# pyannote/pyannote-audio

Hardware: AMD Instinct MI355X
Metric: audio-hours/sec (real-time factor) for speaker-diarization-3.1 pipeline (higher is better)
Workload: dtype f32

## Files before the change

include/pyannote_amd.h:

```cpp
#ifndef PYANNOTE_AMD_H
#define PYANNOTE_AMD_H

#include <stddef.h>
#include <stdint.h>

#ifdef __cplusplus
extern "C" {
#endif

int pa_version(void);
const char* pa_last_error(void);

void pa_prof_enable(int on);
size_t pa_prof_report(char* buf, size_t cap);

#define PA_MAX_LSTM_LAYERS 8
#define PA_MAX_LINEAR 4

typedef struct pa_seg_weights {
  int32_t sinc_stride;
  int32_t lstm_layers;
  int32_t lstm_hidden;
  int32_t lstm_bidir;
  int32_t num_linear;
// ... 27 lines not shown
                   int num_chunks, int num_samples, float* logp, uint8_t* multilabel, void* workspace,
                   size_t workspace_bytes, void* stream);

size_t pa_seg_files_workspace_bytes(const pa_seg_weights* w, int num_files, const int* chunks_per_file,
                                    int num_samples, int64_t chunk_stride);
int pa_seg_forward_files(const pa_seg_weights* w, const float* const* wavs, const int64_t* wav_lens,
                         const int* chunks_per_file, int num_files, int64_t chunk_stride, int num_samples,
                         float* logp, uint8_t* multilabel, void* workspace, size_t workspace_bytes, void* stream);

int pa_row_stats(const float* x, long row_stride, long total_len, int rows, int len, float eps,
                 float* mean, float* rstd, void* stream);
int pa_sinc_fir_pool(const float* wav, long wav_len, long chunk_stride, int B, int N, int stride,
                     const float* mean, const float* rstd, float gamma, float beta,
                     const float* filt_packed, float* out, void* stream);
int pa_sinc_fir_span(const float* wav, long wav_len, long span, const float* filt_packed, float* S, void* stream);
int pa_sinc_fix_pool(const float* S, long Pc, int positions_per_chunk_step, int B, int P, const float* mean,
                     const float* rstd, float gamma, float beta, const float* filt_packed, float* tap_sums,
                     float* out, void* stream);
int pa_sinc_fir_span_centred(const float* wav, long wav_len, long span, const float* mean0, const float* rstd0,
                             const float* filt_packed, float* S, void* stream);
int pa_sinc_fix_pool_centred(const float* S, long Pc, int positions_per_chunk_step, int B, int P, const float* wav,
                             long wav_len, int N, const float* mean, const float* rstd, float gamma, float beta,
                             const float* filt_packed, float* tap_sums, float* out, void* stream);
int pa_conv5_pool(const float* xin, int B, int cin, int Lin, const float* in_mean,
                  const float* in_rstd, const float* gam, const float* bet, const float* w_packed,
                  const float* bias64, float* out, void* stream);
int pa_norm_transpose(const float* xin, int B, int T, const float* in_mean, const float* in_rstd,
                      const float* gam, const float* bet, float* X0, void* stream);
int pa_gemm_tn_ex(const float* A, int lda, const float* W, int ldw, const float* bias, const float* Res,
                  float* C, long ldc, int M, int N, int K, int act, int out_mode, void* stream);
int pa_gemm_tn(const float* A, int lda, const float* W, int ldw, const float* bias, float* C, long ldc,
               int M, int N, int K, int act, int out_mode, void* stream);
int pa_gemm_tn_s2(const float* X, int B, int H, int W, int cin, const float* Wt, int ldw, const float* bias, float* C,
                  long ldc, int N, void* stream);
int pa_lstm_rec(const float* xproj, const float* whh_packed, float* out, int ntiles, int ndir, int T,
                void* stream);
int pa_lstm_rec_h(const float* xproj, const float* whh_packed, float* out, int ntiles, int ndir, int T, int H,
                  void* stream);
int pa_classifier(const float* X, int ldx, int K, int ntiles, int T, int B, const float* cw,
                  const float* cb, int NC, const unsigned char* mapping, int S, float* logp,
                  unsigned char* multilabel, void* stream);

#define PA_MAX_RES_BLOCKS 128

typedef struct pa_emb_weights {
  int32_t num_mel;
// ... 384 lines not shown
```

pyannote-audio_amd/csrc/forward_common.cpp:

```cpp
#include "forward_common.h"

#include <stdlib.h>

namespace pa {

bool sincnet_frames(int sinc_stride, int N, SincNetPlan* p) {
  p->L1 = (N - 251) / sinc_stride + 1;
  if (N < 251 || p->L1 < 3) return false;
  p->P1 = p->L1 / 3;
  if (p->P1 < 5) return false;
  p->P2 = (p->P1 - 4) / 3;
  if (p->P2 < 5) return false;
  p->T = (p->P2 - 4) / 3;
  return p->T >= 1;
}

bool sincnet_plan(int sinc_stride, int B, int N, Bump* ws, SincNetPlan* p) {
  if (!sincnet_frames(sinc_stride, N, p)) return false;
  p->wav_mean = ws->take(B);
  p->wav_rstd = ws->take(B);
  p->s1 = ws->take((size_t)B * 80 * p->P1);
  p->st1m = ws->take((size_t)B * 80);
  p->st1r = ws->take((size_t)B * 80);
  p->s2 = ws->take((size_t)B * 60 * p->P2);
// ... 4 lines not shown
  p->st3r = ws->take((size_t)B * 60);
  p->span = p->span_pos = 0;
  p->span_s = p->tap_sums = 0;
  return true;
}

void sincnet_plan_span(int sinc_stride, int B, int N, int64_t chunk_stride, Bump* ws, SincNetPlan* p) {
  const char* e = getenv("PA_SEG_SHARED_SINC");
  if ((e == nullptr || atoi(e) != 0) && sinc_stride == 10 && B >= 2 && chunk_stride > 0 && chunk_stride < N &&
      chunk_stride % 10 == 0 && (int64_t)(B - 1) * chunk_stride + N <= 0x7fffffffLL) {
    p->span = (long)(B - 1) * chunk_stride + N;
    p->span_pos = (p->span - 251) / 10 + 1;
    p->span_s = ws->take((size_t)80 * p->span_pos);
    p->tap_sums = ws->take(80);
  }
}

int sincnet_sinc_stage(const SincNetView& w, const SincNetPlan& p, const float* wav, int64_t wav_len,
                       int64_t chunk_stride, int B, int N, float* ws, void* stream) {
  PA_RUN(pa_row_stats(wav, chunk_stride, wav_len, B, N, 1e-5f, ws + p.wav_mean, ws + p.wav_rstd, stream));
  if (p.span_pos > 0) {
    PA_RUN(pa_sinc_fir_span_centred(wav, wav_len, p.span, ws + p.wav_mean, ws + p.wav_rstd, w.sinc_filt,
                                    ws + p.span_s, stream));
    PA_RUN(pa_sinc_fix_pool_centred(ws + p.span_s, p.span_pos, (int)(chunk_stride / 10), B, p.P1, wav, wav_len, N,
                                    ws + p.wav_mean, ws + p.wav_rstd, w.wav_gamma, w.wav_beta, w.sinc_filt,
                                    ws + p.tap_sums, ws + p.s1, stream));
  } else {
    PA_RUN(pa_sinc_fir_pool(wav, wav_len, chunk_stride, B, N, w.sinc_stride, ws + p.wav_mean, ws + p.wav_rstd,
                            w.wav_gamma, w.wav_beta, w.sinc_filt, ws + p.s1, stream));
  }
  return 0;
}

int sincnet_after_sinc(const SincNetView& w, const SincNetPlan& p, int B, float* ws, float* x0, void* stream) {
  PA_RUN(pa_row_stats(ws + p.s1, p.P1, (long)B * 80 * p.P1, B * 80, p.P1, 1e-5f, ws + p.st1m, ws + p.st1r, stream));
  PA_RUN(pa_conv5_pool(ws + p.s1, B, 80, p.P1, ws + p.st1m, ws + p.st1r, w.norm0, w.norm0 + 80, w.conv1_w, w.conv1_b,
                       ws + p.s2, stream));
  PA_RUN(pa_row_stats(ws + p.s2, p.P2, (long)B * 60 * p.P2, B * 60, p.P2, 1e-5f, ws + p.st2m, ws + p.st2r, stream));
  PA_RUN(pa_conv5_pool(ws + p.s2, B, 60, p.P2, ws + p.st2m, ws + p.st2r, w.norm1, w.norm1 + 60, w.conv2_w, w.conv2_b,
                       ws + p.s3, stream));
  PA_RUN(pa_row_stats(ws + p.s3, p.T, (long)B * 60 * p.T, B * 60, p.T, 1e-5f, ws + p.st3m, ws + p.st3r, stream));
  return pa_norm_transpose(ws + p.s3, B, p.T, ws + p.st3m, ws + p.st3r, w.norm2, w.norm2 + 60, x0, stream);
}

int sincnet_run(const SincNetView& w, const SincNetPlan& p, const float* wav, int64_t wav_len, int64_t chunk_stride,
                int B, int N, float* ws, float* x0, void* stream) {
  PA_RUN(sincnet_sinc_stage(w, p, wav, wav_len, chunk_stride, B, N, ws, stream));
  return sincnet_after_sinc(w, p, B, ws, x0, stream);
}

bool lstm_head_check(const LstmHeadView& w, const char* who) {
  if (w.lstm_hidden < 16 || w.lstm_hidden % 16 != 0 || w.lstm_hidden > 512 ||
      (!w.lstm_bidir && w.lstm_hidden % 32 != 0) || w.lstm_layers < 1 || w.lstm_layers > PA_MAX_LSTM_LAYERS ||
      w.num_linear > PA_MAX_LINEAR || (w.num_linear > 0 && (w.linear_hidden < 32 || w.linear_hidden % 32 != 0))) {
    set_error("%s: LSTM hidden size must be a multiple of 16 (32 when unidirectional) up to 512, "
              "Linear widths multiples of 32 (got %d, %d)", who, w.lstm_hidden, w.linear_hidden);
    return false;
  }
  return true;
}

void lstm_head_plan(const LstmHeadView& w, int B, int T, Bump* ws, LstmHeadPlan* p) {
  p->ntiles = num_tiles(B);
  p->M = tile_rows(B, T);
  const size_t nd = w.lstm_bidir ? 2 : 1, Hh = (size_t)w.lstm_hidden;
  const size_t lw = w.num_linear > 0 ? (size_t)w.linear_hidden : 0;
  p->xproj = ws->take((size_t)p->M * nd * 4 * Hh);
  p->h0 = ws->take((size_t)p->M * nd * Hh);
  p->h1 = ws->take((size_t)p->M * nd * Hh);
  p->l0 = ws->take((size_t)p->M * lw);
  p->l1 = ws->take((size_t)p->M * lw);
// ... 27 lines not shown
```

pyannote-audio_amd/csrc/forward_common.h:

```cpp
#pragma once
#include <hip/hip_runtime.h>
#include <stdint.h>

#include "../../include/pyannote_amd.h"
#include "common.h"

#define PA_RUN(call)                \
  do {                              \
    const int rc__ = (call);        \
    if (rc__ != 0) return rc__;     \
  } while (0)

namespace pa {

struct Bump {
  size_t o = 0;
  static size_t align(size_t n) { return (n + 63) & ~(size_t)63; }
  size_t take(size_t n) {
    const size_t r = o;
    o += align(n);
    return r;
  }
};

// ... 2 lines not shown

struct SincNetView {
  int sinc_stride;
  float wav_gamma, wav_beta;
  const float *sinc_filt, *norm0, *conv1_w, *conv1_b, *norm1, *conv2_w, *conv2_b, *norm2;
};
template <class W>
SincNetView sincnet_of(const W* w) {
  return {w->sinc_stride, w->wav_gamma, w->wav_beta, w->sinc_filt, w->norm0, w->conv1_w,
          w->conv1_b,     w->norm1,     w->conv2_w,  w->conv2_b,   w->norm2};
}

struct SincNetPlan {
  int L1, P1, P2, T;
  size_t wav_mean, wav_rstd, s1, st1m, st1r, s2, st2m, st2r, s3, st3m, st3r;
  long span, span_pos;
  size_t span_s, tap_sums;
};
PA_INTERNAL bool sincnet_frames(int sinc_stride, int N, SincNetPlan* p);
PA_INTERNAL bool sincnet_plan(int sinc_stride, int B, int N, Bump* ws, SincNetPlan* p);
PA_INTERNAL void sincnet_plan_span(int sinc_stride, int B, int N, int64_t chunk_stride, Bump* ws, SincNetPlan* p);
PA_INTERNAL int sincnet_sinc_stage(const SincNetView& w, const SincNetPlan& p, const float* wav, int64_t wav_len,
                                   int64_t chunk_stride, int B, int N, float* ws, void* stream);
PA_INTERNAL int sincnet_after_sinc(const SincNetView& w, const SincNetPlan& p, int B, float* ws, float* x0,
                                   void* stream);
PA_INTERNAL int sincnet_run(const SincNetView& w, const SincNetPlan& p, const float* wav, int64_t wav_len,
                            int64_t chunk_stride, int B, int N, float* ws, float* x0, void* stream);

struct LstmHeadView {
  int lstm_layers, lstm_hidden, lstm_bidir, num_linear, linear_hidden, num_classes, num_speakers;
  const float* const* lstm_wih;
  const float* const* lstm_bias;
  const float* const* lstm_whh;
  const float* const* lin_w;
  const float* const* lin_b;
  const float *cls_w, *cls_b;
  const uint8_t* powerset_map;
};
template <class W>
LstmHeadView lstm_head_of(const W* w) {
  return {w->lstm_layers, w->lstm_hidden, w->lstm_bidir, w->num_linear, w->linear_hidden, w->num_classes,
          w->num_speakers, w->lstm_wih,   w->lstm_bias,  w->lstm_whh,   w->lin_w,         w->lin_b,
          w->cls_w,        w->cls_b,      w->powerset_map};
}

struct LstmHeadPlan {
  int ntiles;
  long M;
// ... 9 lines not shown
```

pyannote-audio_amd/csrc/seg_forward.cpp:

```cpp
#include "forward_common.h"

namespace {

struct SegPlan {
  pa::SincNetPlan sinc;
  pa::LstmHeadPlan head;
  size_t x0, total;
};

bool make_plan(const pa_seg_weights* w, int B, int N, int64_t chunk_stride, SegPlan* p) {
  pa::Bump ws;
  if (!pa::sincnet_plan(w->sinc_stride, B, N, &ws, &p->sinc)) return false;
  p->x0 = ws.take((size_t)pa::tile_rows(B, p->sinc.T) * 64);
  pa::lstm_head_plan(pa::lstm_head_of(w), B, p->sinc.T, &ws, &p->head);
  pa::sincnet_plan_span(w->sinc_stride, B, N, chunk_stride, &ws, &p->sinc);
  p->total = ws.o;
  return true;
}

struct FilesPlan {
  SegPlan seg;
  long chunks;
  size_t span_base;
};
// ... 86 lines not shown
                         float* logp, uint8_t* multilabel, void* workspace, size_t workspace_bytes, void* stream) {
  FilesPlan p;
  const int bad = make_files_plan(w, num_files, chunks_per_file, num_samples, chunk_stride, &p);
  if (bad == 1) {
    pa::set_error("pa_seg_forward_files: a negative chunk count, or more than 65535 chunks in one launch group");
    return 3;
  }
  if (bad != 0) {
    pa::set_error("pa_seg_forward_files: chunk of %d samples is too short for SincNet", num_samples);
    return 3;
  }
  if (p.chunks == 0) return 0;
  const pa::LstmHeadView head = pa::lstm_head_of(w);
  if (!pa::lstm_head_check(head, "pa_seg_forward_files")) return 3;
  if (workspace_bytes < p.seg.total * sizeof(float)) {
    pa::set_error("pa_seg_forward_files: workspace too small (%zu < %zu bytes)", workspace_bytes,
                  p.seg.total * sizeof(float));
    return 3;
  }
  float* ws = (float*)workspace;
  const pa::SincNetView sinc = pa::sincnet_of(w);
  const int B = (int)p.chunks;
  long c0 = 0;
  for (int f = 0; f < num_files; ++f) {
    const int Bf = chunks_per_file[f];
    if (Bf == 0) continue;
    pa::SincNetPlan one = p.seg.sinc;
    one.wav_mean += c0;
    one.wav_rstd += c0;
    one.s1 += (size_t)c0 * 80 * one.P1;
    plan_file_span(w, Bf, num_samples, chunk_stride, p.span_base, &one);
    PA_RUN(pa::sincnet_sinc_stage(sinc, one, wavs[f], wav_lens[f], chunk_stride, Bf, num_samples, ws, stream));
    c0 += Bf;
  }
  PA_RUN(pa::sincnet_after_sinc(sinc, p.seg.sinc, B, ws, ws + p.seg.x0, stream));
  return pa::lstm_head_run(head, p.seg.head, ws + p.seg.x0, 64, B, p.seg.sinc.T, ws, logp, multilabel, stream);
}

}
```

pyannote-audio_amd/csrc/seg_frontend.hip:

```cpp
#include "common.h"

namespace pa {

__global__ __launch_bounds__(256) void k_row_stats(const float* __restrict__ x, long row_stride,
                                                    long total_len, int len, float eps,
                                                    float* __restrict__ mean_out,
                                                    float* __restrict__ rstd_out) {
  __shared__ float red[4];
  const long base = (long)blockIdx.x * row_stride;
  long avail = total_len - base;
  int valid = avail >= len ? len : (avail > 0 ? (int)avail : 0);
  const float* row = x + base;
  float s = 0.f;
  for (int i = threadIdx.x; i < valid; i += 256) s += row[i];
  const float mean = block_sum<4>(s, red) / (float)len;
  float q = 0.f;
  for (int i = threadIdx.x; i < valid; i += 256) {
    float d = row[i] - mean;
    q += d * d;
  }
  float var = block_sum<4>(q, red);
  var += (float)(len - valid) * mean * mean;
  var /= (float)len;
  if (threadIdx.x == 0) {
    mean_out[blockIdx.x] = mean;
    rstd_out[blockIdx.x] = 1.0f / sqrtf(var + eps);
  }
}

constexpr int SINC_PT = 128;
constexpr int SINC_XS = 30 * SINC_PT + 256;
constexpr int SINC_OS = SINC_PT + 4;
constexpr int SINC_T = 640;
constexpr float SINC_DEMOTE = 0.5f;

__device__ __forceinline__ float sinc_centre(float mean0, float rstd0) {
  return fabsf(mean0) * rstd0 > SINC_DEMOTE ? mean0 : 0.f;
}
__device__ __forceinline__ bool sinc_demoted(float mu, float rstd, float m0) {
  return fabsf(mu - m0) * rstd > SINC_DEMOTE;
}

template <bool RAW, int STR = 10>
__global__ __launch_bounds__(SINC_T) void k_sinc_fir_pool(
    const float* __restrict__ wav, long wav_len, long chunk_stride, int N, int stride, int P,
    const float* __restrict__ mean, const float* __restrict__ rstd, float gamma, float beta,
    const float* __restrict__ filt, float* __restrict__ out, int centred) {
  constexpr int XS_MAX = 3 * STR * SINC_PT + 256;
  extern __shared__ __attribute__((aligned(16))) float smem[];
  float* xs = smem;
  float* os = smem + XS_MAX;
  const int b = blockIdx.y;
  const int p0 = blockIdx.x * SINC_PT;
  const int tid = threadIdx.x, lane = tid & 63;
  const int w = (tid >> 6) % 5, half = (tid >> 6) / 5;
  constexpr int PS = RAW ? STR : 3 * STR;
  constexpr int XS = RAW ? STR * SINC_PT + 256 : XS_MAX;

  const long cbase = (long)b * chunk_stride;
  if (!RAW && centred && !sinc_demoted(mean[b], rstd[b], sinc_centre(mean[0], rstd[0]))) return;
  const float mu = RAW ? (centred ? sinc_centre(mean[0], rstd[0]) : 0.f) : mean[b], rs = RAW ? 1.f : rstd[b] * gamma;
  if (RAW) beta = 0.f;
  {
    constexpr int NS = (XS_MAX + SINC_T - 1) / SINC_T;
// ... 31 lines not shown
#pragma unroll
    for (int r = 0; r < 4; ++r) {
      const float v = RAW ? a0[r] : fmaxf(fmaxf(fabsf(a0[r]), fabsf(a1[r])), fabsf(a2[r]));
      os[(16 * w + i16) * SINC_OS + 16 * grp + 4 * kq + r] = v;
    }
  }
  __syncthreads();
  const int np = min(SINC_PT, P - p0);
  for (int i = tid; i < 80 * SINC_PT; i += SINC_T) {
    const int c = i / SINC_PT, p = i % SINC_PT;
    if (p < np) out[((long)b * 80 + c) * P + p0 + p] = os[c * SINC_OS + p];
  }
}

__global__ __launch_bounds__(128) void k_sinc_tapsum(const float* __restrict__ filt, float* __restrict__ S1) {
  const int f = threadIdx.x;
  if (f >= 80) return;
  double acc = 0.0;
  for (int kt = 0; kt < 63; ++kt)
    for (int q = 0; q < 4; ++q) acc += (double)filt[((f >> 4) * 63 + kt) * 64 + (f & 15) + 16 * q];
  S1[f] = (float)acc;
}

__global__ __launch_bounds__(256) void k_sinc_fix_pool(const float* __restrict__ S, long Pc, int Q, int P,
                                                        const float* __restrict__ mean,
                                                        const float* __restrict__ rstd, float gamma, float beta,
                                                        const float* __restrict__ S1, float* __restrict__ out,
                                                        int centred) {
  const int b = blockIdx.y, p = blockIdx.x * 256 + threadIdx.x;
  if (p >= P) return;
  const float m0 = centred ? sinc_centre(mean[0], rstd[0]) : 0.f;
  if (centred && sinc_demoted(mean[b], rstd[b], m0)) return;
  const float mu = mean[b] - m0, g = rstd[b] * gamma;
  const float* src = S + (long)b * Q + 3 * p;
  float* dst = out + (long)b * 80 * P + p;
#pragma unroll 8
  for (int f = 0; f < 80; ++f) {
    const float s1 = S1[f], off = beta * s1 - g * mu * s1;
    const float* row = src + (long)f * Pc;
    const float v0 = fabsf(fmaf(g, row[0], off)), v1 = fabsf(fmaf(g, row[1], off)), v2 = fabsf(fmaf(g, row[2], off));
    dst[(long)f * P] = fmaxf(fmaxf(v0, v1), v2);
  }
}

constexpr int CV_PT = 32;
constexpr int CV_XW = 112;
constexpr int CV_OS = CV_PT + 1;

template <int CIN>
__global__ __launch_bounds__(256) void k_conv5_pool(const float* __restrict__ xin, int Lin, int P,
                                                     const float* __restrict__ in_mean,
                                                     const float* __restrict__ in_rstd,
                                                     const float* __restrict__ gam,
                                                     const float* __restrict__ bet,
                                                     const float* __restrict__ wp,
                                                     const float* __restrict__ bias,
                                                     float* __restrict__ out) {
  constexpr int KT = 5 * CIN / 4;
  constexpr int KPT = CIN / 4;
  __shared__ __attribute__((aligned(16))) float xs[CIN * CV_XW];
  __shared__ float os[64 * CV_OS];
  const int b = blockIdx.y;
  const int p0 = blockIdx.x * CV_PT;
  const int tid = threadIdx.x, lane = tid & 63, w = tid >> 6;
// ... 74 lines not shown
      const int row = b * 60 + c;
      v = (xin[(long)row * T + t0 + tt] - in_mean[row]) * (in_rstd[row] * gam[c]) + bet[c];
      v = leaky_relu(v);
    }
    tile[c][tt] = v;
  }
  __syncthreads();
  const int bt = b >> 4, b16 = b & 15;
  for (int i = tid; i < 64 * 64; i += 256) {
    const int tt = i >> 6, c = i & 63;
    if (t0 + tt < T) X0[(((long)bt * T + t0 + tt) * 16 + b16) * 64 + c] = tile[c][tt];
  }
}

}

extern "C" {

int pa_row_stats(const float* x, long row_stride, long total_len, int rows, int len, float eps,
                 float* mean, float* rstd, void* stream) {
  if (rows <= 0) return 0;
  pa::ProfScope prof("k_row_stats", stream, 5.0 * rows * len, 8.0 * rows * len);
  hipLaunchKernelGGL(pa::k_row_stats, dim3(rows), dim3(256), 0, (hipStream_t)stream, x, row_stride,
                     total_len, len, eps, mean, rstd);
  PA_CHECK_LAUNCH("pa_row_stats");
  return 0;
}

int pa_sinc_fir_pool(const float* wav, long wav_len, long chunk_stride, int B, int N, int stride,
                     const float* mean, const float* rstd, float gamma, float beta,
                     const float* filt_packed, float* out, void* stream) {
  PA_REQUIRE(stride >= 1 && N >= 251, "pa_sinc_fir_pool: stride %d / %d samples", stride, N);
  const int L = (N - 251) / stride + 1;
  const int P = L / 3;
  if (B <= 0 || P <= 0) return 0;
  pa::ProfScope prof("k_sinc_fir_pool", stream, 2.0 * B * 80 * 251 * (3.0 * P),
                     4.0 * B * N + 4.0 * B * 80 * P);
#define PA_SINC_LAUNCH(S)                                                                                          \
  do {                                                                                                             \
    const size_t lds = (size_t)(3 * (S) * pa::SINC_PT + 256 + 80 * pa::SINC_OS) * sizeof(float);                     \
                         \
    (void)hipFuncSetAttribute((const void*)pa::k_sinc_fir_pool<false, S>, hipFuncAttributeMaxDynamicSharedMemorySize, \
                              (int)lds);                                                                           \
    hipLaunchKernelGGL((pa::k_sinc_fir_pool<false, S>), dim3(pa::cdiv(P, pa::SINC_PT), B), dim3(pa::SINC_T), lds,  \
                       (hipStream_t)stream, wav, wav_len, chunk_stride, N, stride, P, mean, rstd, gamma, beta,      \
                       filt_packed, out, 0);                                                                       \
  } while (0)
// ... 54 lines not shown

int pa_sinc_fix_pool_centred(const float* S, long Pc, int positions_per_chunk_step, int B, int P, const float* wav,
                             long wav_len, int N, const float* mean, const float* rstd, float gamma, float beta,
                             const float* filt_packed, float* tap_sums, float* out, void* stream) {
  if (B <= 0 || P <= 0) return 0;
  PA_REQUIRE(N >= 251 && P == ((N - 251) / 10 + 1) / 3, "pa_sinc_fix_pool_centred: %d pooled positions of %d samples",
             P, N);
  pa::ProfScope prof("k_sinc_fix_pool", stream, 8.0 * B * 80 * 3.0 * P, 4.0 * B * 80 * 4.0 * P);
  hipLaunchKernelGGL(pa::k_sinc_tapsum, dim3(1), dim3(128), 0, (hipStream_t)stream, filt_packed, tap_sums);
  hipLaunchKernelGGL(pa::k_sinc_fix_pool, dim3(pa::cdiv(P, 256), B), dim3(256), 0, (hipStream_t)stream, S, Pc,
                     positions_per_chunk_step, P, mean, rstd, gamma, beta, (const float*)tap_sums, out, 1);
  {
    const size_t lds = (pa::SINC_XS + 80 * pa::SINC_OS) * sizeof(float);
    (void)hipFuncSetAttribute((const void*)pa::k_sinc_fir_pool<false, 10>, hipFuncAttributeMaxDynamicSharedMemorySize,
                              (int)lds);
    hipLaunchKernelGGL((pa::k_sinc_fir_pool<false, 10>), dim3(pa::cdiv(P, pa::SINC_PT), B), dim3(pa::SINC_T), lds,
                       (hipStream_t)stream, wav, wav_len, 10L * positions_per_chunk_step, N, 10, P, mean, rstd, gamma,
                       beta, filt_packed, out, 1);
  }
  PA_CHECK_LAUNCH("pa_sinc_fix_pool_centred");
  return 0;
}

int pa_conv5_pool(const float* xin, int B, int cin, int Lin, const float* in_mean,
                  const float* in_rstd, const float* gam, const float* bet, const float* w_packed,
                  const float* bias64, float* out, void* stream) {
  const int P = (Lin - 4) / 3;
  if (B <= 0 || P <= 0) return 0;
  dim3 grid(pa::cdiv(P, pa::CV_PT), B);
  pa::ProfScope prof("k_conv5_pool", stream, 2.0 * B * 60 * cin * 5 * (3.0 * P),
                     4.0 * B * cin * Lin + 4.0 * B * 60 * P);
  if (cin == 80)
    hipLaunchKernelGGL(pa::k_conv5_pool<80>, grid, dim3(256), 0, (hipStream_t)stream, xin, Lin, P,
                       in_mean, in_rstd, gam, bet, w_packed, bias64, out);
  else if (cin == 60)
    hipLaunchKernelGGL(pa::k_conv5_pool<60>, grid, dim3(256), 0, (hipStream_t)stream, xin, Lin, P,
                       in_mean, in_rstd, gam, bet, w_packed, bias64, out);
  else
    PA_REQUIRE(false, "pa_conv5_pool: unsupported cin %d", cin);
  PA_CHECK_LAUNCH("pa_conv5_pool");
  return 0;
}

int pa_norm_transpose(const float* xin, int B, int T, const float* in_mean, const float* in_rstd,
                      const float* gam, const float* bet, float* X0, void* stream) {
  if (B <= 0) return 0;
// ... 10 lines not shown
```

pyannote-audio_amd/csrc/seg_lstm.hip:

```cpp
#include "common.h"

namespace pa {

constexpr int GB = 128;
constexpr int GK = 32;
constexpr int GLD = GK + 4;

template <int ACT, int OUT_MODE>
__global__ __launch_bounds__(256) void k_gemm_tn(const float* __restrict__ A, int lda,
                                                  const float* __restrict__ W, int ldw,
                                                  const float* __restrict__ bias,
                                                  const float* __restrict__ Res,
                                                  float* __restrict__ C, long ldc, int M, int N, int K,
                                                  int nm, int nn, int inner, long sAo, long sAi, long sWo,
                                                  long sWi, long sCo, long sCi, int gHW, int gWo, int gH, int gW) {
  if (gridDim.y > 1) {
    const int zo = blockIdx.y / inner, zi = blockIdx.y % inner;
    A += zo * sAo + zi * sAi;
    W += zo * sWo + zi * sWi;
    C += zo * sCo + zi * sCi;
    if (Res != nullptr) Res += zo * sCo + zi * sCi;
  }
  __shared__ __attribute__((aligned(16))) float As[GB * GLD];
  __shared__ __attribute__((aligned(16))) float Ws[GB * GLD];
// ... 263 lines not shown
      for (int mt = 0; mt < MT; ++mt) {
        float* hn = hsg + ((mt * 2 + (cur ^ 1)) * 16 + 4 * g) * hstride + 16 * u + n;
        float* op = out + (((long)tl[mt] * T + t) * 16 + 4 * g) * ldo + dir * H + 16 * u + n;
#pragma unroll
        for (int r = 0; r < 4; ++r) {
          const float ig = sigmoidf_(acc[mt][0][r] + xin[mt][0][r]);
          const float fg = sigmoidf_(acc[mt][1][r] + xin[mt][1][r]);
          const float gg = tanhf_(acc[mt][2][r] + xin[mt][2][r]);
          const float og = sigmoidf_(acc[mt][3][r] + xin[mt][3][r]);
          const float cn = fg * c[ui][mt][r] + ig * gg;
          c[ui][mt][r] = cn;
          const float h = og * tanhf_(cn);
          hn[r * hstride] = h;
          if (live[mt]) op[(long)r * ldo] = h;
        }
      }
    }
    __syncthreads();
    cur ^= 1;
  }
}

constexpr int CLS_MAXC = 16;

__global__ __launch_bounds__(256) void k_classifier(const float* __restrict__ X, int ldx, int K, int M,
                                                     int T, int B, const float* __restrict__ cw,
                                                     const float* __restrict__ cb, int NC,
                                                     const unsigned char* __restrict__ mapping, int S,
                                                     float* __restrict__ logp,
                                                     unsigned char* __restrict__ ml) {
  extern __shared__ float wsh[];
  for (int i = threadIdx.x; i < NC * K; i += 256) wsh[i] = cw[i];
  for (int i = threadIdx.x; i < NC; i += 256) wsh[NC * K + i] = cb[i];
  __syncthreads();
  const long m = (long)blockIdx.x * 256 + threadIdx.x;
  if (m >= M) return;
  const int b16 = (int)(m & 15);
  const long tt = m >> 4;
  const int t = (int)(tt % T), tile = (int)(tt / T);
  const int b = tile * 16 + b16;
  if (b >= B) return;
  float z[CLS_MAXC];
#pragma unroll
  for (int cidx = 0; cidx < CLS_MAXC; ++cidx) z[cidx] = cidx < NC ? wsh[NC * K + cidx] : 0.f;
  const float* x = X + m * ldx;
  for (int k = 0; k < K; k += 4) {
    const float4 xv = *reinterpret_cast<const float4*>(x + k);
#pragma unroll
    for (int cidx = 0; cidx < CLS_MAXC; ++cidx)
      if (cidx < NC) {
        const float* wrow = wsh + cidx * K + k;
        z[cidx] = fmaf(xv.x, wrow[0], z[cidx]);
        z[cidx] = fmaf(xv.y, wrow[1], z[cidx]);
        z[cidx] = fmaf(xv.z, wrow[2], z[cidx]);
        z[cidx] = fmaf(xv.w, wrow[3], z[cidx]);
      }
  }
  const long o = (long)b * T + t;
  if (mapping == nullptr) {
    if (logp != nullptr)
      for (int cidx = 0; cidx < NC; ++cidx) logp[o * NC + cidx] = 1.f / (1.f + expf(-z[cidx]));
    return;
  }
  float mx = z[0];
  int am = 0;
#pragma unroll
  for (int cidx = 1; cidx < CLS_MAXC; ++cidx)
    if (cidx < NC && z[cidx] > mx) {
      mx = z[cidx];
      am = cidx;
    }
  float se = 0.f;
#pragma unroll
  for (int cidx = 0; cidx < CLS_MAXC; ++cidx)
    if (cidx < NC) se += expf(z[cidx] - mx);
  const float lse = mx + logf(se);
  if (logp != nullptr)
    for (int cidx = 0; cidx < NC; ++cidx) logp[o * NC + cidx] = z[cidx] - lse;
  if (ml != nullptr)
// ... 111 lines not shown
    static size_t granted = 0;
    if (lds > granted) {
      PA_REQUIRE(hipFuncSetAttribute((const void*)pa::k_lstm_rec_gen, hipFuncAttributeMaxDynamicSharedMemorySize,
                                     (int)lds) == hipSuccess,
                 "pa_lstm_rec_h: cannot reserve %zu bytes of dynamic LDS for hidden size %d", lds, H);
      granted = lds;
    }
  }
  pa::ProfScope prof("k_lstm_rec_gen", stream, 2.0 * ntiles * 16 * ndir * T * H * 4.0 * H,
                     4.0 * ntiles * 16 * ndir * T * (4.0 * H + H));
  hipLaunchKernelGGL(pa::k_lstm_rec_gen, dim3(pa::cdiv(ntiles, pa::LSTMG_MT), ndir), dim3(256), lds,
                     (hipStream_t)stream, xproj, whh_packed, out, T, H, ntiles, ndir, hstride);
  PA_CHECK_LAUNCH("pa_lstm_rec_h");
  return 0;
}

int pa_classifier(const float* X, int ldx, int K, int ntiles, int T, int B, const float* cw,
                  const float* cb, int NC, const unsigned char* mapping, int S, float* logp,
                  unsigned char* multilabel, void* stream) {
  PA_REQUIRE(NC <= pa::CLS_MAXC && K % 4 == 0, "pa_classifier: NC <= 16 and K %% 4 == 0 required");
  const long M = (long)ntiles * T * 16;
  if (M <= 0) return 0;
  const size_t lds = (size_t)(NC * K + NC) * sizeof(float);
  pa::ProfScope prof("k_classifier", stream, 2.0 * M * K * NC, 4.0 * M * K + 4.0 * M * NC);
  hipLaunchKernelGGL(pa::k_classifier, dim3(pa::cdiv(M, 256)), dim3(256), lds, (hipStream_t)stream, X,
                     ldx, K, (int)M, T, B, cw, cb, NC, mapping, S, logp, multilabel);
  PA_CHECK_LAUNCH("pa_classifier");
  return 0;
}

}
```

pyannote-audio_amd/ffi.py:

```python
from __future__ import annotations

import ctypes as C
from pathlib import Path

import torch

_LIB = None
PA_MAX_LSTM_LAYERS = 8
PA_MAX_LINEAR = 4

c_fp = C.c_void_p


class SegWeights(C.Structure):
    _fields_ = [
        ("sinc_stride", C.c_int32), ("lstm_layers", C.c_int32), ("lstm_hidden", C.c_int32),
        ("lstm_bidir", C.c_int32), ("num_linear", C.c_int32), ("linear_hidden", C.c_int32),
        ("num_classes", C.c_int32), ("num_speakers", C.c_int32),
        ("wav_gamma", C.c_float), ("wav_beta", C.c_float),
        ("sinc_filt", c_fp), ("norm0", c_fp), ("conv1_w", c_fp), ("conv1_b", c_fp), ("norm1", c_fp),
        ("conv2_w", c_fp), ("conv2_b", c_fp), ("norm2", c_fp),
        ("lstm_wih", c_fp * PA_MAX_LSTM_LAYERS), ("lstm_bias", c_fp * PA_MAX_LSTM_LAYERS),
        ("lstm_whh", c_fp * PA_MAX_LSTM_LAYERS),
        ("lin_w", c_fp * PA_MAX_LINEAR), ("lin_b", c_fp * PA_MAX_LINEAR),
# ... 143 lines not shown
    lib.pa_prof_report.restype = C.c_size_t
    _declare_optional(lib)
    _LIB = lib
    return lib


_OPTIONAL: list[tuple] = [
    ("pa_emb_num_fbank_frames", [C.c_int], C.c_int),
    ("pa_emb_num_pool_frames", [C.POINTER(EmbWeights), C.c_int], C.c_int),
    ("pa_emb_workspace_bytes", [C.POINTER(EmbWeights), C.c_int, C.c_int, C.c_int], C.c_size_t),
    ("pa_emb_forward", [C.POINTER(EmbWeights), c_fp, C.c_int64, C.c_int64, C.c_int, C.c_int, c_fp,
                        C.c_int, C.c_int, c_fp, c_fp, c_fp, C.c_size_t, c_fp], C.c_int),
    ("pa_emb_ragged_workspace_bytes", [C.POINTER(EmbWeights), C.c_int, C.c_int], C.c_size_t),
    ("pa_emb_forward_ragged", [C.POINTER(EmbWeights), c_fp, C.c_int64, c_fp, c_fp, C.c_int, C.c_int, c_fp, c_fp,
                               c_fp, C.c_size_t, c_fp], C.c_int),
    ("pa_fbank_ragged", [c_fp, C.c_long, c_fp, c_fp, C.c_int, C.c_int, c_fp, c_fp, c_fp, c_fp, c_fp, c_fp, C.c_int,
                         c_fp, c_fp], C.c_int),
    ("pa_zero_tail_cols", [c_fp, C.c_int, C.c_int, C.c_int, C.c_int, c_fp, C.c_int, c_fp], C.c_int),
    ("pa_stats_pool_ragged", [c_fp, C.c_int, C.c_int, C.c_int, C.c_int, c_fp, C.c_int, c_fp, C.c_int, c_fp, c_fp],
     C.c_int),
    ("pa_emb_calibrate_workspace_bytes", [C.POINTER(EmbWeights), C.c_int, C.c_int], C.c_size_t),
    ("pa_emb_calibrate_winograd", [C.POINTER(EmbWeights), c_fp, C.c_int64, C.c_int64, C.c_int, C.c_int, c_fp, c_fp,
                                   c_fp, C.c_size_t, c_fp], C.c_int),
    ("pa_lstm_rec_h", [c_fp, c_fp, c_fp, C.c_int, C.c_int, C.c_int, C.c_int, c_fp], C.c_int),
    ("pa_absmax_diff", [c_fp, c_fp, C.c_long, c_fp, c_fp], C.c_int),
    ("pa_gemm_tn_s2", [c_fp, C.c_int, C.c_int, C.c_int, C.c_int, c_fp, C.c_int, c_fp, c_fp, C.c_long, C.c_int,
                       c_fp], C.c_int),
    ("pa_gemm_tn_batched", [c_fp, C.c_int, C.c_long, C.c_long, c_fp, C.c_int, C.c_long, C.c_long, c_fp, c_fp, C.c_long,
                            C.c_long, C.c_long, C.c_int, C.c_int, C.c_int, C.c_int, C.c_int, C.c_int, c_fp], C.c_int),
    ("pa_fbank", [c_fp, C.c_long, C.c_long, C.c_int, C.c_int, c_fp, c_fp, c_fp, c_fp, c_fp, c_fp,
                  C.c_int, c_fp, C.c_int, c_fp], C.c_int),
    ("pa_fbank_center_span", [c_fp, C.c_int, C.c_int, C.c_int, C.c_int, c_fp, c_fp], C.c_int),
    ("pa_resnet_stem", [c_fp, C.c_int, C.c_int, C.c_int, c_fp, c_fp, c_fp, c_fp], C.c_int),
    ("pa_conv3x3", [c_fp, C.c_int, C.c_int, C.c_int, C.c_int, c_fp, c_fp, c_fp, c_fp, C.c_int, C.c_int,
                    C.c_int, c_fp], C.c_int),
    ("pa_conv3x3_s2_sc_supported", [C.c_int, C.c_int, C.c_int], C.c_int),
    ("pa_conv3x3_s2_sc", [c_fp, C.c_int, C.c_int, C.c_int, C.c_int, c_fp, c_fp, c_fp, c_fp, c_fp, c_fp, C.c_int,
                          C.c_int, c_fp], C.c_int),
    ("pa_conv3x3_wino", [c_fp, C.c_int, C.c_int, C.c_int, C.c_int, c_fp, c_fp, c_fp, c_fp, C.c_int, C.c_int,
                         c_fp], C.c_int),
    ("pa_conv3x3_wino4", [c_fp, C.c_int, C.c_int, C.c_int, C.c_int, c_fp, c_fp, c_fp, c_fp, C.c_int, C.c_int,
                          c_fp], C.c_int),
    ("pa_conv3x3_wino4_rows", [c_fp, C.c_int, C.c_int, C.c_int, C.c_int, c_fp, c_fp, c_fp, c_fp, C.c_int, C.c_int,
                               C.c_int, c_fp], C.c_int),
    ("pa_conv3x3_wino_rows", [c_fp, C.c_int, C.c_int, C.c_int, C.c_int, c_fp, c_fp, c_fp, c_fp, C.c_int, C.c_int,
                              C.c_int, c_fp], C.c_int),
# ... 173 lines not shown
```

Measured before the change: 1.342.

## Fuse sinc pooling with row statistics, register-cache row stats, stage classifier inputs

Adds a sinc fix-pool kernel that also computes the per-row mean and rstd of its pooled output, so the separate row-stats pass over the first SincNet activation is skipped on the shared-span path. The row-stats kernel now caches each row in registers for one read, and can skip rows that do not need recomputing after the demoted-chunk fallback. The classifier kernel stages input tiles through LDS so loads from global memory are coalesced. These changes add more kernel variants and more register pressure, and the demoted-chunk path has to recompute stats to stay correct.

```diff
diff --git a/include/pyannote_amd.h b/include/pyannote_amd.h
--- a/include/pyannote_amd.h
+++ b/include/pyannote_amd.h
@@ -73,6 +73,13 @@
 int pa_sinc_fix_pool_centred(const float* S, long Pc, int positions_per_chunk_step, int B, int P, const float* wav,
                              long wav_len, int N, const float* mean, const float* rstd, float gamma, float beta,
                              const float* filt_packed, float* tap_sums, float* out, void* stream);
+int pa_sinc_fix_pool_stats(const float* S, long Pc, int positions_per_chunk_step, int B, int P, const float* mean,
+                           const float* rstd, float gamma, float beta, const float* filt_packed, float* tap_sums,
+                           float* out, float eps, float* st_mean, float* st_rstd, void* stream);
+int pa_sinc_fix_pool_stats_centred(const float* S, long Pc, int positions_per_chunk_step, int B, int P,
+                                   const float* wav, long wav_len, int N, const float* mean, const float* rstd,
+                                   float gamma, float beta, const float* filt_packed, float* tap_sums, float* out,
+                                   float eps, float* st_mean, float* st_rstd, void* stream);
 int pa_conv5_pool(const float* xin, int B, int cin, int Lin, const float* in_mean,
                   const float* in_rstd, const float* gam, const float* bet, const float* w_packed,
                   const float* bias64, float* out, void* stream);
diff --git a/pyannote-audio_amd/csrc/forward_common.cpp b/pyannote-audio_amd/csrc/forward_common.cpp
--- a/pyannote-audio_amd/csrc/forward_common.cpp
+++ b/pyannote-audio_amd/csrc/forward_common.cpp
@@ -50,9 +50,9 @@
   if (p.span_pos > 0) {
     PA_RUN(pa_sinc_fir_span_centred(wav, wav_len, p.span, ws + p.wav_mean, ws + p.wav_rstd, w.sinc_filt,
                                     ws + p.span_s, stream));
-    PA_RUN(pa_sinc_fix_pool_centred(ws + p.span_s, p.span_pos, (int)(chunk_stride / 10), B, p.P1, wav, wav_len, N,
-                                    ws + p.wav_mean, ws + p.wav_rstd, w.wav_gamma, w.wav_beta, w.sinc_filt,
-                                    ws + p.tap_sums, ws + p.s1, stream));
+    PA_RUN(pa_sinc_fix_pool_stats_centred(ws + p.span_s, p.span_pos, (int)(chunk_stride / 10), B, p.P1, wav, wav_len, N,
+                                          ws + p.wav_mean, ws + p.wav_rstd, w.wav_gamma, w.wav_beta, w.sinc_filt,
+                                          ws + p.tap_sums, ws + p.s1, 1e-5f, ws + p.st1m, ws + p.st1r, stream));
   } else {
     PA_RUN(pa_sinc_fir_pool(wav, wav_len, chunk_stride, B, N, w.sinc_stride, ws + p.wav_mean, ws + p.wav_rstd,
                             w.wav_gamma, w.wav_beta, w.sinc_filt, ws + p.s1, stream));
@@ -60,8 +60,11 @@
   return 0;
 }
 
-int sincnet_after_sinc(const SincNetView& w, const SincNetPlan& p, int B, float* ws, float* x0, void* stream) {
-  PA_RUN(pa_row_stats(ws + p.s1, p.P1, (long)B * 80 * p.P1, B * 80, p.P1, 1e-5f, ws + p.st1m, ws + p.st1r, stream));
+int sincnet_after_sinc(const SincNetView& w, const SincNetPlan& p, int B, bool have_st1, float* ws, float* x0,
+                       void* stream) {
+  if (!have_st1)
+    PA_RUN(pa_row_stats(ws + p.s1, p.P1, (long)B * 80 * p.P1, B * 80, p.P1, 1e-5f, ws + p.st1m, ws + p.st1r,
+                        stream));
   PA_RUN(pa_conv5_pool(ws + p.s1, B, 80, p.P1, ws + p.st1m, ws + p.st1r, w.norm0, w.norm0 + 80, w.conv1_w, w.conv1_b,
                        ws + p.s2, stream));
   PA_RUN(pa_row_stats(ws + p.s2, p.P2, (long)B * 60 * p.P2, B * 60, p.P2, 1e-5f, ws + p.st2m, ws + p.st2r, stream));
@@ -74,7 +77,7 @@
 int sincnet_run(const SincNetView& w, const SincNetPlan& p, const float* wav, int64_t wav_len, int64_t chunk_stride,
                 int B, int N, float* ws, float* x0, void* stream) {
   PA_RUN(sincnet_sinc_stage(w, p, wav, wav_len, chunk_stride, B, N, ws, stream));
-  return sincnet_after_sinc(w, p, B, ws, x0, stream);
+  return sincnet_after_sinc(w, p, B, sincnet_has_st1(p), ws, x0, stream);
 }
 
 bool lstm_head_check(const LstmHeadView& w, const char* who) {
diff --git a/pyannote-audio_amd/csrc/forward_common.h b/pyannote-audio_amd/csrc/forward_common.h
--- a/pyannote-audio_amd/csrc/forward_common.h
+++ b/pyannote-audio_amd/csrc/forward_common.h
@@ -48,8 +48,9 @@
 PA_INTERNAL void sincnet_plan_span(int sinc_stride, int B, int N, int64_t chunk_stride, Bump* ws, SincNetPlan* p);
 PA_INTERNAL int sincnet_sinc_stage(const SincNetView& w, const SincNetPlan& p, const float* wav, int64_t wav_len,
                                    int64_t chunk_stride, int B, int N, float* ws, void* stream);
-PA_INTERNAL int sincnet_after_sinc(const SincNetView& w, const SincNetPlan& p, int B, float* ws, float* x0,
-                                   void* stream);
+inline bool sincnet_has_st1(const SincNetPlan& p) { return p.span_pos > 0; }
+PA_INTERNAL int sincnet_after_sinc(const SincNetView& w, const SincNetPlan& p, int B, bool have_st1, float* ws,
+                                   float* x0, void* stream);
 PA_INTERNAL int sincnet_run(const SincNetView& w, const SincNetPlan& p, const float* wav, int64_t wav_len,
                             int64_t chunk_stride, int B, int N, float* ws, float* x0, void* stream);
 
diff --git a/pyannote-audio_amd/csrc/seg_forward.cpp b/pyannote-audio_amd/csrc/seg_forward.cpp
--- a/pyannote-audio_amd/csrc/seg_forward.cpp
+++ b/pyannote-audio_amd/csrc/seg_forward.cpp
@@ -132,6 +132,7 @@
   const pa::SincNetView sinc = pa::sincnet_of(w);
   const int B = (int)p.chunks;
   long c0 = 0;
+  bool have_st1 = true;
   for (int f = 0; f < num_files; ++f) {
     const int Bf = chunks_per_file[f];
     if (Bf == 0) continue;
@@ -139,11 +140,14 @@
     one.wav_mean += c0;
     one.wav_rstd += c0;
     one.s1 += (size_t)c0 * 80 * one.P1;
+    one.st1m += (size_t)c0 * 80;
+    one.st1r += (size_t)c0 * 80;
     plan_file_span(w, Bf, num_samples, chunk_stride, p.span_base, &one);
+    have_st1 = have_st1 && pa::sincnet_has_st1(one);
     PA_RUN(pa::sincnet_sinc_stage(sinc, one, wavs[f], wav_lens[f], chunk_stride, Bf, num_samples, ws, stream));
     c0 += Bf;
   }
-  PA_RUN(pa::sincnet_after_sinc(sinc, p.seg.sinc, B, ws, ws + p.seg.x0, stream));
+  PA_RUN(pa::sincnet_after_sinc(sinc, p.seg.sinc, B, have_st1, ws, ws + p.seg.x0, stream));
   return pa::lstm_head_run(head, p.seg.head, ws + p.seg.x0, 64, B, p.seg.sinc.T, ws, logp, multilabel, stream);
 }
 
diff --git a/pyannote-audio_amd/csrc/seg_frontend.hip b/pyannote-audio_amd/csrc/seg_frontend.hip
--- a/pyannote-audio_amd/csrc/seg_frontend.hip
+++ b/pyannote-audio_amd/csrc/seg_frontend.hip
@@ -1,26 +1,75 @@
 #include "common.h"
 
 namespace pa {
+
+constexpr float SINC_DEMOTE = 0.5f;
+__device__ __forceinline__ float sinc_centre(float mean0, float rstd0) {
+  return fabsf(mean0) * rstd0 > SINC_DEMOTE ? mean0 : 0.f;
+}
+__device__ __forceinline__ bool sinc_demoted(float mu, float rstd, float m0) {
+  return fabsf(mu - m0) * rstd > SINC_DEMOTE;
+}
+
+constexpr int RS_NV = 24;
+
+template <int NV>
+__device__ __forceinline__ void row_stats_once(const float* __restrict__ row, int valid, int len, float* red,
+                                               float& mean, float& var) {
+  float v[NV];
+#pragma unroll
+  for (int k = 0; k < NV; ++k) {
+    const int i = threadIdx.x + 256 * k;
+    v[k] = i < valid ? row[i] : 0.f;
+  }
+  float s = 0.f;
+#pragma unroll
+  for (int k = 0; k < NV; ++k)
+    if ((int)threadIdx.x + 256 * k < valid) s += v[k];
+  mean = block_sum<4>(s, red) / (float)len;
+  float q = 0.f;
+#pragma unroll
+  for (int k = 0; k < NV; ++k)
+    if ((int)threadIdx.x + 256 * k < valid) {
+      float d = v[k] - mean;
+      q = fmaf(d, d, q);
+    }
+  var = block_sum<4>(q, red);
+}
 
 __global__ __launch_bounds__(256) void k_row_stats(const float* __restrict__ x, long row_stride,
                                                     long total_len, int len, float eps,
                                                     float* __restrict__ mean_out,
-                                                    float* __restrict__ rstd_out) {
+                                                    float* __restrict__ rstd_out,
+                                                    const float* __restrict__ chunk_mean,
+                                                    const float* __restrict__ chunk_rstd, int rows_per_chunk) {
   __shared__ float red[4];
+  if (chunk_mean != nullptr) {
+    const int b = blockIdx.x / rows_per_chunk;
+    if (!sinc_demoted(chunk_mean[b], chunk_rstd[b], sinc_centre(chunk_mean[0], chunk_rstd[0]))) return;
+  }
   const long base = (long)blockIdx.x * row_stride;
   long avail = total_len - base;
   int valid = avail >= len ? len : (avail > 0 ? (int)avail : 0);
   const float* row = x + base;
-  float s = 0.f;
-  for (int i = threadIdx.x; i < valid; i += 256) s += row[i];
-  const float mean = block_sum<4>(s, red) / (float)len;
-  float q = 0.f;
-  for (int i = threadIdx.x; i < valid; i += 256) {
-    float d = row[i] - mean;
-    q += d * d;
-  }
-  float var = block_sum<4>(q, red);
-  var += (float)(len - valid) * mean * mean;
+  float mean, var;
+  if (len <= 256 * 4) {
+    row_stats_once<4>(row, valid, len, red, mean, var);
+  } else if (len <= 256 * 8) {
+    row_stats_once<8>(row, valid, len, red, mean, var);
+  } else if (len <= 256 * RS_NV) {
+    row_stats_once<RS_NV>(row, valid, len, red, mean, var);
+  } else {
+    float s = 0.f;
+    for (int i = threadIdx.x; i < valid; i += 256) s += row[i];
+    mean = block_sum<4>(s, red) / (float)len;
+    float q = 0.f;
+    for (int i = threadIdx.x; i < valid; i += 256) {
+      float d = row[i] - mean;
+      q = fmaf(d, d, q);
+    }
+    var = block_sum<4>(q, red);
+  }
+  var = fmaf((float)(len - valid) * mean, mean, var);
   var /= (float)len;
   if (threadIdx.x == 0) {
     mean_out[blockIdx.x] = mean;
@@ -32,14 +81,6 @@
 constexpr int SINC_XS = 30 * SINC_PT + 256;
 constexpr int SINC_OS = SINC_PT + 4;
 constexpr int SINC_T = 640;
-constexpr float SINC_DEMOTE = 0.5f;
-
-__device__ __forceinline__ float sinc_centre(float mean0, float rstd0) {
-  return fabsf(mean0) * rstd0 > SINC_DEMOTE ? mean0 : 0.f;
-}
-__device__ __forceinline__ bool sinc_demoted(float mu, float rstd, float m0) {
-  return fabsf(mu - m0) * rstd > SINC_DEMOTE;
-}
 
 template <bool RAW, int STR = 10>
 __global__ __launch_bounds__(SINC_T) void k_sinc_fir_pool(
@@ -117,6 +158,12 @@
   S1[f] = (float)acc;
 }
 
+__device__ __forceinline__ float sinc_fix_offset(float beta, float g, float mu, float s1) {
+#pragma clang fp contract(off)
+  const float a = beta * s1, c = g * mu * s1;
+  return a - c;
+}
+
 __global__ __launch_bounds__(256) void k_sinc_fix_pool(const float* __restrict__ S, long Pc, int Q, int P,
                                                         const float* __restrict__ mean,
                                                         const float* __restrict__ rstd, float gamma, float beta,
@@ -131,10 +178,69 @@
   float* dst = out + (long)b * 80 * P + p;
 #pragma unroll 8
   for (int f = 0; f < 80; ++f) {
-    const float s1 = S1[f], off = beta * s1 - g * mu * s1;
+    const float off = sinc_fix_offset(beta, g, mu, S1[f]);
     const float* row = src + (long)f * Pc;
     const float v0 = fabsf(fmaf(g, row[0], off)), v1 = fabsf(fmaf(g, row[1], off)), v2 = fabsf(fmaf(g, row[2], off));
     dst[(long)f * P] = fmaxf(fmaxf(v0, v1), v2);
+  }
+}
+
+constexpr int SFS_NV = 24;
+constexpr int SFS_G = 8;
+
+__global__ __launch_bounds__(256) void k_sinc_fix_pool_stats(const float* __restrict__ S, long Pc, int Q, int P,
+                                                              const float* __restrict__ mean,
+                                                              const float* __restrict__ rstd, float gamma, float beta,
+                                                              const float* __restrict__ S1, float* __restrict__ out,
+                                                              int centred, float eps, float* __restrict__ st_mean,
+                                                              float* __restrict__ st_rstd) {
+  __shared__ float red[4];
+  const int b = blockIdx.x / 80, f = blockIdx.x % 80;
+  const float m0 = centred ? sinc_centre(mean[0], rstd[0]) : 0.f;
+  if (centred && sinc_demoted(mean[b], rstd[b], m0)) return;
+  const float mu = mean[b] - m0, g = rstd[b] * gamma;
+  const float off = sinc_fix_offset(beta, g, mu, S1[f]);
+  const float* src = S + (long)f * Pc + (long)b * Q;
+  float* dst = out + ((long)b * 80 + f) * P;
+  float v[SFS_NV];
+  float s = 0.f;
+#pragma unroll
+  for (int k0 = 0; k0 < SFS_NV; k0 += SFS_G) {
+    if (256 * k0 >= P) break;
+    float r[SFS_G][3];
+#pragma unroll
+    for (int k = 0; k < SFS_G; ++k) {
+      const int p = threadIdx.x + 256 * (k0 + k);
+      const float* row = src + 3 * p;
+#pragma unroll
+      for (int j = 0; j < 3; ++j) r[k][j] = p < P ? row[j] : 0.f;
+    }
+#pragma unroll
+    for (int k = 0; k < SFS_G; ++k) {
+      const int p = threadIdx.x + 256 * (k0 + k);
+      const float v0 = fabsf(fmaf(g, r[k][0], off)), v1 = fabsf(fmaf(g, r[k][1], off)),
+                  v2 = fabsf(fmaf(g, r[k][2], off));
+      v[k0 + k] = fmaxf(fmaxf(v0, v1), v2);
+      if (p < P) {
+        dst[p] = v[k0 + k];
+        s += v[k0 + k];
+      }
+    }
+  }
+  const float mean_row = block_sum<4>(s, red) / (float)P;
+  float q = 0.f;
+#pragma unroll
+  for (int k = 0; k < SFS_NV; ++k)
+    if ((int)threadIdx.x + 256 * k < P) {
+      float d = v[k] - mean_row;
+      q = fmaf(d, d, q);
+    }
+  float var = block_sum<4>(q, red);
+  var = fmaf(0.f * mean_row, mean_row, var);
+  var /= (float)P;
+  if (threadIdx.x == 0) {
+    st_mean[blockIdx.x] = mean_row;
+    st_rstd[blockIdx.x] = 1.0f / sqrtf(var + eps);
   }
 }
 
@@ -255,7 +361,7 @@
   if (rows <= 0) return 0;
   pa::ProfScope prof("k_row_stats", stream, 5.0 * rows * len, 8.0 * rows * len);
   hipLaunchKernelGGL(pa::k_row_stats, dim3(rows), dim3(256), 0, (hipStream_t)stream, x, row_stride,
-                     total_len, len, eps, mean, rstd);
+                     total_len, len, eps, mean, rstd, (const float*)nullptr, (const float*)nullptr, 1);
   PA_CHECK_LAUNCH("pa_row_stats");
   return 0;
 }
@@ -356,6 +462,57 @@
   return 0;
 }
 
+static int sinc_fix_pool_stats(const float* S, long Pc, int step, int B, int P, const float* wav, long wav_len, int N,
+                               const float* mean, const float* rstd, float gamma, float beta, const float* filt_packed,
+                               float* tap_sums, float* out, float eps, float* st_mean, float* st_rstd, int centred,
+                               void* stream) {
+  if (P > 256 * pa::SFS_NV) {
+    const int rc = centred ? pa_sinc_fix_pool_centred(S, Pc, step, B, P, wav, wav_len, N, mean, rstd, gamma, beta,
+                                                      filt_packed, tap_sums, out, stream)
+                           : pa_sinc_fix_pool(S, Pc, step, B, P, mean, rstd, gamma, beta, filt_packed, tap_sums, out,
+                                              stream);
+    if (rc != 0) return rc;
+    return pa_row_stats(out, P, (long)B * 80 * P, B * 80, P, eps, st_mean, st_rstd, stream);
+  }
+  PA_REQUIRE((long)B * 80 <= 0x7fffffffL, "pa_sinc_fix_pool_stats: %d chunks are too many", B);
+  pa::ProfScope prof("k_sinc_fix_pool_stats", stream, 8.0 * B * 80 * 3.0 * P + 5.0 * B * 80 * P,
+                     4.0 * B * 80 * 4.0 * P);
+  hipLaunchKernelGGL(pa::k_sinc_tapsum, dim3(1), dim3(128), 0, (hipStream_t)stream, filt_packed, tap_sums);
+  hipLaunchKernelGGL(pa::k_sinc_fix_pool_stats, dim3(B * 80), dim3(256), 0, (hipStream_t)stream, S, Pc, step, P, mean,
+                     rstd, gamma, beta, (const float*)tap_sums, out, centred, eps, st_mean, st_rstd);
+  if (centred) {
+    const size_t lds = (pa::SINC_XS + 80 * pa::SINC_OS) * sizeof(float);
+    (void)hipFuncSetAttribute((const void*)pa::k_sinc_fir_pool<false, 10>, hipFuncAttributeMaxDynamicSharedMemorySize,
+                              (int)lds);
+    hipLaunchKernelGGL((pa::k_sinc_fir_pool<false, 10>), dim3(pa::cdiv(P, pa::SINC_PT), B), dim3(pa::SINC_T), lds,
+                       (hipStream_t)stream, wav, wav_len, 10L * step, N, 10, P, mean, rstd, gamma, beta, filt_packed,
+                       out, 1);
+    hipLaunchKernelGGL(pa::k_row_stats, dim3(B * 80), dim3(256), 0, (hipStream_t)stream, (const float*)out, (long)P,
+                       (long)B * 80 * P, P, eps, st_mean, st_rstd, mean, rstd, 80);
+  }
+  PA_CHECK_LAUNCH("pa_sinc_fix_pool_stats");
+  return 0;
+}
+
+int pa_sinc_fix_pool_stats(const float* S, long Pc, int positions_per_chunk_step, int B, int P, const float* mean,
+                           const float* rstd, float gamma, float beta, const float* filt_packed, float* tap_sums,
+                           float* out, float eps, float* st_mean, float* st_rstd, void* stream) {
+  if (B <= 0 || P <= 0) return 0;
+  return sinc_fix_pool_stats(S, Pc, positions_per_chunk_step, B, P, nullptr, 0, 0, mean, rstd, gamma, beta,
+                             filt_packed, tap_sums, out, eps, st_mean, st_rstd, 0, stream);
+}
+
+int pa_sinc_fix_pool_stats_centred(const float* S, long Pc, int positions_per_chunk_step, int B, int P,
+                                   const float* wav, long wav_len, int N, const float* mean, const float* rstd,
+                                   float gamma, float beta, const float* filt_packed, float* tap_sums, float* out,
+                                   float eps, float* st_mean, float* st_rstd, void* stream) {
+  if (B <= 0 || P <= 0) return 0;
+  PA_REQUIRE(N >= 251 && P == ((N - 251) / 10 + 1) / 3,
+             "pa_sinc_fix_pool_stats_centred: %d pooled positions of %d samples", P, N);
+  return sinc_fix_pool_stats(S, Pc, positions_per_chunk_step, B, P, wav, wav_len, N, mean, rstd, gamma, beta,
+                             filt_packed, tap_sums, out, eps, st_mean, st_rstd, 1, stream);
+}
+
 int pa_conv5_pool(const float* xin, int B, int cin, int Lin, const float* in_mean,
                   const float* in_rstd, const float* gam, const float* bet, const float* w_packed,
                   const float* bias64, float* out, void* stream) {
diff --git a/pyannote-audio_amd/csrc/seg_lstm.hip b/pyannote-audio_amd/csrc/seg_lstm.hip
--- a/pyannote-audio_amd/csrc/seg_lstm.hip
+++ b/pyannote-audio_amd/csrc/seg_lstm.hip
@@ -309,7 +309,10 @@
 }
 
 constexpr int CLS_MAXC = 16;
-
+constexpr int CLS_KB = 32;
+constexpr int CLS_XS = CLS_KB + 1;
+
+template <bool STAGED>
 __global__ __launch_bounds__(256) void k_classifier(const float* __restrict__ X, int ldx, int K, int M,
                                                      int T, int B, const float* __restrict__ cw,
                                                      const float* __restrict__ cb, int NC,
@@ -321,27 +324,67 @@
   for (int i = threadIdx.x; i < NC; i += 256) wsh[NC * K + i] = cb[i];
   __syncthreads();
   const long m = (long)blockIdx.x * 256 + threadIdx.x;
-  if (m >= M) return;
   const int b16 = (int)(m & 15);
   const long tt = m >> 4;
   const int t = (int)(tt % T), tile = (int)(tt / T);
   const int b = tile * 16 + b16;
-  if (b >= B) return;
+  const bool live = m < M && b < B;
+  if (!STAGED && !live) return;
   float z[CLS_MAXC];
 #pragma unroll
   for (int cidx = 0; cidx < CLS_MAXC; ++cidx) z[cidx] = cidx < NC ? wsh[NC * K + cidx] : 0.f;
-  const float* x = X + m * ldx;
-  for (int k = 0; k < K; k += 4) {
-    const float4 xv = *reinterpret_cast<const float4*>(x + k);
-#pragma unroll
-    for (int cidx = 0; cidx < CLS_MAXC; ++cidx)
-      if (cidx < NC) {
-        const float* wrow = wsh + cidx * K + k;
-        z[cidx] = fmaf(xv.x, wrow[0], z[cidx]);
-        z[cidx] = fmaf(xv.y, wrow[1], z[cidx]);
-        z[cidx] = fmaf(xv.z, wrow[2], z[cidx]);
-        z[cidx] = fmaf(xv.w, wrow[3], z[cidx]);
-      }
+  if (STAGED) {
+    float* xs = wsh + ((NC * K + NC + 3) & ~3);
+    const int sr = threadIdx.x >> 3, sc = (threadIdx.x & 7) * 4;
+    const long mb = (long)blockIdx.x * 256;
+    for (int k0 = 0; k0 < K; k0 += CLS_KB) {
+      const int kb = min(CLS_KB, K - k0);
+      float4 xr[8];
+#pragma unroll
+      for (int i = 0; i < 8; ++i) {
+        const long r = mb + sr + 32 * i;
+        xr[i] = (r < M && sc < kb) ? *reinterpret_cast<const float4*>(X + r * ldx + k0 + sc)
+                                   : make_float4(0.f, 0.f, 0.f, 0.f);
+      }
+      __syncthreads();
+#pragma unroll
+      for (int i = 0; i < 8; ++i) {
+        float* d = xs + (sr + 32 * i) * CLS_XS + sc;
+        d[0] = xr[i].x;
+        d[1] = xr[i].y;
+        d[2] = xr[i].z;
+        d[3] = xr[i].w;
+      }
+      __syncthreads();
+      const float* xrow = xs + threadIdx.x * CLS_XS;
+      for (int k = 0; k < kb; k += 4) {
+        const float x0 = xrow[k], x1 = xrow[k + 1], x2 = xrow[k + 2], x3 = xrow[k + 3];
+#pragma unroll
+        for (int cidx = 0; cidx < CLS_MAXC; ++cidx)
+          if (cidx < NC) {
+            const float* wrow = wsh + cidx * K + k0 + k;
+            z[cidx] = fmaf(x0, wrow[0], z[cidx]);
+            z[cidx] = fmaf(x1, wrow[1], z[cidx]);
+            z[cidx] = fmaf(x2, wrow[2], z[cidx]);
+            z[cidx] = fmaf(x3, wrow[3], z[cidx]);
+          }
+      }
+    }
+    if (!live) return;
+  } else {
+    const float* x = X + m * ldx;
+    for (int k = 0; k < K; k += 4) {
+      const float4 xv = *reinterpret_cast<const float4*>(x + k);
+#pragma unroll
+      for (int cidx = 0; cidx < CLS_MAXC; ++cidx)
+        if (cidx < NC) {
+          const float* wrow = wsh + cidx * K + k;
+          z[cidx] = fmaf(xv.x, wrow[0], z[cidx]);
+          z[cidx] = fmaf(xv.y, wrow[1], z[cidx]);
+          z[cidx] = fmaf(xv.z, wrow[2], z[cidx]);
+          z[cidx] = fmaf(xv.w, wrow[3], z[cidx]);
+        }
+    }
   }
   const long o = (long)b * T + t;
   if (mapping == nullptr) {
@@ -499,9 +542,14 @@
   const long M = (long)ntiles * T * 16;
   if (M <= 0) return 0;
   const size_t lds = (size_t)(NC * K + NC) * sizeof(float);
+  const size_t lds_staged = (size_t)(((NC * K + NC + 3) & ~3) + 256 * pa::CLS_XS) * sizeof(float);
   pa::ProfScope prof("k_classifier", stream, 2.0 * M * K * NC, 4.0 * M * K + 4.0 * M * NC);
-  hipLaunchKernelGGL(pa::k_classifier, dim3(pa::cdiv(M, 256)), dim3(256), lds, (hipStream_t)stream, X,
-                     ldx, K, (int)M, T, B, cw, cb, NC, mapping, S, logp, multilabel);
+  if (lds_staged <= 64 * 1024)
+    hipLaunchKernelGGL(pa::k_classifier<true>, dim3(pa::cdiv(M, 256)), dim3(256), lds_staged, (hipStream_t)stream, X,
+                       ldx, K, (int)M, T, B, cw, cb, NC, mapping, S, logp, multilabel);
+  else
+    hipLaunchKernelGGL(pa::k_classifier<false>, dim3(pa::cdiv(M, 256)), dim3(256), lds, (hipStream_t)stream, X,
+                       ldx, K, (int)M, T, B, cw, cb, NC, mapping, S, logp, multilabel);
   PA_CHECK_LAUNCH("pa_classifier");
   return 0;
 }
diff --git a/pyannote-audio_amd/ffi.py b/pyannote-audio_amd/ffi.py
--- a/pyannote-audio_amd/ffi.py
+++ b/pyannote-audio_amd/ffi.py
@@ -189,6 +189,10 @@
     ("pa_emb_calibrate_workspace_bytes", [C.POINTER(EmbWeights), C.c_int, C.c_int], C.c_size_t),
     ("pa_emb_calibrate_winograd", [C.POINTER(EmbWeights), c_fp, C.c_int64, C.c_int64, C.c_int, C.c_int, c_fp, c_fp,
                                    c_fp, C.c_size_t, c_fp], C.c_int),
+    ("pa_sinc_fix_pool_stats", [c_fp, C.c_long, C.c_int, C.c_int, C.c_int, c_fp, c_fp, C.c_float, C.c_float, c_fp, c_fp,
+                                c_fp, C.c_float, c_fp, c_fp, c_fp], C.c_int),
+    ("pa_sinc_fix_pool_stats_centred", [c_fp, C.c_long, C.c_int, C.c_int, C.c_int, c_fp, C.c_long, C.c_int, c_fp, c_fp,
+                                        C.c_float, C.c_float, c_fp, c_fp, c_fp, C.c_float, c_fp, c_fp, c_fp], C.c_int),
     ("pa_lstm_rec_h", [c_fp, c_fp, c_fp, C.c_int, C.c_int, C.c_int, C.c_int, c_fp], C.c_int),
     ("pa_absmax_diff", [c_fp, c_fp, C.c_long, c_fp, c_fp], C.c_int),
     ("pa_gemm_tn_s2", [c_fp, C.c_int, C.c_int, C.c_int, C.c_int, c_fp, C.c_int, c_fp, c_fp, C.c_long, C.c_int,
```

New measurement: 1.351, median of 6. About the same (+0.7%).
